# 1005088h/3d_object_detection

Hardware: AMD Instinct MI355X
Metric: point-cloud frames/sec end-to-end (voxelise→NMS), eight_20cm, 1x MI355X (higher is better)
Workload: dtype f32; 1 GPU; configs/eight_20cm.json, synthetic KITTI-shape 64-beam 20k-point clouds (mean 20000 points, one distinct cloud per frame of a step), independent frames (batch=1 semantics), random-init weights (InstanceNorm backbone), AABB NMS; `value`: clouds resident in HBM; frames_per_pass_per_gpu=32, engine_max_batch=32, parallelism=frame-sharded x1

## Files before the change

3d_object_detection_amd/_lib.py:

```python
import ctypes
import os

_HERE = os.path.dirname(os.path.abspath(__file__))
LIB_PATH = os.path.join(_HERE, "csrc", "libpp_hip.so")
PP_MAX_CLASSES = 12
PP_LOSS_TERMS = 21
PP_ASSIGN_MAX_GT = 4096
PP_AUG_MAX_BOXES = 256
PP_AUG_MAX_TRIES = 128
PP_AUG_PARAMS = 16
PP_OPT_CHUNK = 2048
PP_OPT_GROUP = 32

c_f = ctypes.c_float
c_i32 = ctypes.c_int32
c_i64 = ctypes.c_int64
c_p = ctypes.c_void_p


class PPConfig(ctypes.Structure):
    _fields_ = [
        ("voxel_size", c_f * 3),
        ("offset", c_f * 3),
        ("grid_size", c_i32 * 3),
# ... 12 lines not shown
        ("nms_iou_threshold", c_f),
        ("score_threshold", c_f),
        ("max_batch", c_i32),
    ]


PROTOTYPES = {
    "pp_create": (c_p, [ctypes.c_int, ctypes.POINTER(PPConfig)]),
    "pp_destroy": (None, [c_p]),
    "pp_last_error": (ctypes.c_char_p, [c_p]),
    "pp_load_weights": (ctypes.c_int, [c_p, ctypes.c_char_p, c_p, ctypes.POINTER(c_i64), ctypes.c_int]),
    "pp_commit_weights": (ctypes.c_int, [c_p]),
    "pp_set_precision": (ctypes.c_int, [c_p, ctypes.c_int]),
    "pp_effective_precision": (ctypes.c_int, [c_p]),
    "pp_set_anchors": (ctypes.c_int, [c_p, c_p, c_p, c_i64]),
    "pp_voxelize": (ctypes.c_int, [c_p, c_p, ctypes.c_int, ctypes.c_int, c_p, c_p, c_p, c_p, c_p]),
    "pp_anchor_mask": (ctypes.c_int, [c_p, c_p, c_p, c_p, c_p]),
    "pp_pfn": (ctypes.c_int, [c_p, c_p, c_p, c_p, c_p, c_p, c_p]),
    "pp_scatter": (ctypes.c_int, [c_p, c_p, c_p, c_p, c_p, c_p]),
    "pp_backbone": (ctypes.c_int, [c_p, c_p, c_p, c_p]),
    "pp_head": (ctypes.c_int, [c_p, c_p, c_p, c_p, c_p, c_p]),
    "pp_postprocess": (ctypes.c_int, [c_p, c_p, c_p, c_p, c_p, c_p, c_p, ctypes.c_int, c_p]),
    "pp_select_candidates": (ctypes.c_int, [c_p, c_p, c_p, c_p, c_p, c_p, c_p, c_p, c_p]),
    "pp_infer_frame": (ctypes.c_int, [c_p, c_p, ctypes.c_int, c_p, c_p, ctypes.c_int, c_p]),
    "pp_infer_batch": (ctypes.c_int, [c_p, ctypes.POINTER(c_p), ctypes.POINTER(c_i32), ctypes.c_int, c_p, c_p, ctypes.c_int, c_p]),
    "pp_fetch_frame_tensor": (ctypes.c_int, [c_p, ctypes.c_int, ctypes.c_int, c_p, c_p]),
    "pp_debug_layer": (ctypes.c_int, [c_p, ctypes.c_int, ctypes.c_int, c_p, c_p, ctypes.c_int, c_p, c_p, c_p, c_p, c_p, c_p, c_p, c_p, c_p]),
    "pp_debug_layer_skip": (ctypes.c_int, [c_p, ctypes.c_int, ctypes.c_int, c_p, c_p, ctypes.c_int, c_p, c_p, c_p, c_p, c_p, c_p, c_p, c_p, c_p, ctypes.c_int, c_p]),
    "pp_debug_head_cls": (ctypes.c_int, [c_p, ctypes.c_int, c_p, ctypes.c_int, c_p, c_p, c_p, c_p]),
    "pp_head_cls_tiling": (ctypes.c_char_p, [c_p]),
    "pp_set_head_defer": (ctypes.c_int, [c_p, ctypes.c_int]),
    "pp_head_defer_active": (ctypes.c_int, [c_p]),
    "pp_set_sparse_conv1": (ctypes.c_int, [c_p, ctypes.c_int]),
    "pp_set_tile_skip": (ctypes.c_int, [c_p, ctypes.c_int]),
    "pp_tile_skip_active": (ctypes.c_int, [c_p]),
    "pp_set_assign_thresholds": (ctypes.c_int, [c_p, c_p, c_p]),
    "pp_assign_targets": (ctypes.c_int, [c_p, c_p, c_p, c_p, ctypes.POINTER(c_i32), ctypes.c_int, c_p, c_p, c_p, c_p, c_p]),
    "pp_target_loss": (ctypes.c_int, [c_p, c_p, c_p, c_p, c_p, c_p, c_p, ctypes.c_int, c_p, c_p]),
    "pp_batch_loss": (ctypes.c_int, [c_p, c_p, c_p, ctypes.POINTER(c_i32), ctypes.c_int, c_p, c_p]),
    "pp_target_loss_grad": (ctypes.c_int, [c_p, c_p, c_p, c_p, c_p, c_p, c_p, ctypes.c_int, ctypes.c_int, c_f, c_p, c_p, c_p, c_p]),
    "pp_head_backward": (ctypes.c_int, [c_p, c_p, c_p, c_p, c_p, ctypes.c_int, c_p, c_p, c_p, c_p, c_p, c_p, c_p, c_p]),
    "pp_update_head_weights": (ctypes.c_int, [c_p, c_p, c_p, c_p, c_p, c_p, c_p, c_p]),
    "pp_backbone_taps": (ctypes.c_int, [c_p, c_p, c_p, c_p, c_p, c_p, c_p]),
    "pp_neck_backward": (ctypes.c_int, [c_p, ctypes.c_int, c_p, c_p, c_p, c_p, ctypes.c_int, c_p, c_p, c_p]),
    "pp_update_neck_weights": (ctypes.c_int, [c_p, c_p, c_p, c_p, c_p]),
    "pp_unit_backward": (ctypes.c_int, [c_p, ctypes.c_int, ctypes.c_int, ctypes.c_int, c_p, c_p, c_p, c_p, ctypes.c_int, c_p, c_p, c_p]),
    "pp_unit_backward_mp": (ctypes.c_int, [c_p, ctypes.c_int, ctypes.c_int, ctypes.c_int, ctypes.c_int, c_p, c_p, c_p, c_p, ctypes.c_int, c_p, c_p,
                                           c_p]),
    "pp_unit_backward_path": (ctypes.c_int, [c_p, ctypes.c_int, ctypes.c_int, ctypes.c_int, ctypes.c_int]),
    "pp_backbone_block_taps": (ctypes.c_int, [c_p, c_p, c_p, c_p, c_p, c_p, c_p, c_p]),
    "pp_update_block_weights": (ctypes.c_int, [c_p, ctypes.c_int, c_p, ctypes.c_int, c_p]),
    "pp_down_backward": (ctypes.c_int, [c_p, ctypes.c_int, ctypes.c_int, ctypes.c_int, ctypes.c_int, c_p, c_p, c_p, c_p, ctypes.c_int, c_p, c_p, c_p]),
    "pp_backbone_stage_taps": (ctypes.c_int, [c_p, c_p, c_p, c_p, c_p, c_p, c_p, c_p, c_p]),
    "pp_update_down_weight": (ctypes.c_int, [c_p, ctypes.c_int, c_p, c_p]),
    "pp_backbone_train_taps": (ctypes.c_int, [c_p, c_p, c_p, c_p, c_p, c_p, c_p, c_p, c_p]),
    "pp_update_rpn_weights": (ctypes.c_int, [c_p, c_p, c_p]),
    "pp_unit_backward_affine": (ctypes.c_int, [c_p, ctypes.c_int, ctypes.c_int, ctypes.c_int, c_p, c_p, c_p, c_p, c_p, c_p, ctypes.c_int, c_p, c_p, c_p,
                                               c_p, c_p]),
    "pp_down_backward_affine": (ctypes.c_int, [c_p, ctypes.c_int, ctypes.c_int, ctypes.c_int, ctypes.c_int, c_p, c_p, c_p, c_p, c_p, c_p, ctypes.c_int,
                                               c_p, c_p, c_p, c_p, c_p]),
    "pp_neck_backward_affine": (ctypes.c_int, [c_p, ctypes.c_int, c_p, c_p, c_p, c_p, c_p, c_p, ctypes.c_int, c_p, c_p, c_p, c_p, c_p]),
    "pp_bn_fold": (ctypes.c_int, [c_p, ctypes.c_int, c_p, c_p, c_p, c_p, c_p, c_p, c_p]),
    "pp_bn_affine_grad": (ctypes.c_int, [c_p, ctypes.c_int, c_p, c_p, c_p, c_p, c_p, c_p, c_p]),
    "pp_update_bn_fold": (ctypes.c_int, [c_p, c_p, c_p]),
    "pp_pfn_train_forward": (ctypes.c_int, [c_p] * 12),
    "pp_scatter_backward": (ctypes.c_int, [c_p] * 6),
# ... 65 lines not shown
```

3d_object_detection_amd/csrc/conv_inspect.hip:

```cpp
#include <algorithm>
#include <cstdio>
#include <cstring>
#include "conv_net.h"

using namespace ppc;

static int packed_indices(pp_ctx* ctx, const Layer& L, bool index_positions, std::vector<int32_t>& map)
{
    Layer scratch = L;
    scratch.w = nullptr;
    int rc = pack_layer(ctx, scratch, index_positions);
    if (rc) { if (scratch.w) (void)hipFree(scratch.w); return rc; }
    std::vector<float> image(scratch.w_bytes / sizeof(float));
    const hipError_t e = hipMemcpy(image.data(), scratch.w, scratch.w_bytes, hipMemcpyDeviceToHost);
    (void)hipFree(scratch.w);
    PP_HIP(e);
    map.resize(image.size());
    for (size_t i = 0; i < image.size(); ++i) map[i] = (int32_t)image[i] - 1;
    return 0;
}

static int layer_index_map(pp_ctx* ctx, const Layer& L, const std::vector<std::string>& names, std::vector<int32_t>& wmap)
{
    std::vector<std::vector<float>> saved(names.size());
// ... 86 lines not shown
        return 0;
    }
    return pp_fail(ctx, PP_E_ARG, "pp_net_deconv_image: no such upsampler");
}

extern "C" int pp_fetch_frame_tensor(pp_ctx* ctx, int frame, int kind, void* dst, void* stream_)
{
    if (!ctx || !dst) return pp_fail(ctx, PP_E_ARG, "pp_fetch_frame_tensor: null pointer");
    if (frame < 0 || frame >= ctx->max_batch) return pp_fail(ctx, PP_E_ARG, "pp_fetch_frame_tensor: frame out of range");
    hipStream_t stream = (hipStream_t)stream_;
    pp_net* net = (pp_net*)ctx->net;
    const size_t A = (size_t)ctx->A, mv = (size_t)ctx->cfg.max_voxels, HW = (size_t)ctx->H * ctx->W;
    const void* src = nullptr;
    size_t bytes = 0;
    if (kind == 1 || kind == 2)
        if (int rc0 = pp_head_materialise(ctx, stream)) return rc0;
    switch (kind) {
    case 0: src = ctx->f_cls + frame * A; bytes = A * 4; break;
    case 1: src = ctx->f_box + frame * A * 7; bytes = A * 28; break;
    case 2: src = ctx->f_dir + frame * A * 2; bytes = A * 8; break;
    case 3: src = ctx->f_mask + frame * A; bytes = A; break;
    case 4: {
        NormRef pre = norm_ref(ctx, 7, 320, 0, HW);
        if (pre.mode == PRE_STATS) pre.acc += (size_t)frame * STAT_FS;
        const float* src_ = net->up16 ? reinterpret_cast<const float*>(reinterpret_cast<const _Float16*>(net->up) + (size_t)frame * 320 * HW)
                                      : net->up + (size_t)frame * 320 * HW;
        return launch_norm_relu(ctx, src_, (float*)dst, 320, (int)HW, pre, nullptr, stream, 1, net->up16 ? 1 : 0);
    }
    case 5: src = ctx->f_feat + frame * mv * 64; bytes = mv * 64 * 4; break;
    case 6: src = ctx->f_coors + frame * mv * 3; bytes = mv * 12; break;
    case 7: src = ctx->f_num + frame * 4; bytes = 4; break;
    case 8: return pp_sc1_fetch_list(ctx, frame, dst, stream);
    case 9: return pp_ts_fetch_flags(ctx, frame, dst, stream);
    default: return pp_fail(ctx, PP_E_ARG, "pp_fetch_frame_tensor: unknown kind");
    }
    PP_HIP(hipMemcpyAsync(dst, src, bytes, hipMemcpyDeviceToDevice, stream));
    return 0;
}

namespace {
__global__ void __launch_bounds__(256) dbg_reduce_stats(const double* __restrict__ acc, size_t acc_fs, int C, double* __restrict__ out)
{
    const int i = blockIdx.x * 256 + threadIdx.x;
    if (i >= 2 * C) return;
    const double* a = acc + (size_t)blockIdx.y * acc_fs;
    double s = 0.0;
#pragma unroll
    for (int r = 0; r < NREP; ++r) s += a[(size_t)r * C * 2 + i];
    out[(size_t)blockIdx.y * 2 * C + i] = s;
}
}

extern "C" int pp_debug_layer(pp_ctx* ctx, int layer, int nb, const void* in, const void* res, int pre_mode, const float* scale, const float* shift,
                              const int32_t* pmap, const float* feat, void* out, float* out_box, float* out_dir, double* stats, void* stream_)
{
    return pp_debug_layer_skip(ctx, layer, nb, in, res, pre_mode, scale, shift, pmap, feat, out, out_box, out_dir, stats, nullptr, 0, stream_);
}

extern "C" int pp_debug_layer_skip(pp_ctx* ctx, int layer, int nb, const void* in, const void* res, int pre_mode, const float* scale, const float* shift,
                                   const int32_t* pmap, const float* feat, void* out, float* out_box, float* out_dir, double* stats,
                                   const uint8_t* active, int skip_k, void* stream_)
{
    if (!ctx) return PP_E_ARG;
    if (!ctx->net || !ctx->weights_ready) return pp_fail(ctx, PP_E_STATE, "pp_debug_layer: weights not committed");
    pp_net* net = (pp_net*)ctx->net;
    if (layer < 0 || layer >= (int)net->layers.size()) return pp_fail(ctx, PP_E_ARG, "pp_debug_layer: layer index out of range");
// ... 201 lines not shown
```

3d_object_detection_amd/csrc/conv_run.hip:

```cpp
#include <cstring>
#include "conv_net.h"

namespace ppc {
namespace {

__global__ void __launch_bounds__(256) norm_relu_stats(const float* __restrict__ x, float* __restrict__ y, int C, int HW,
                                                       int pre, const double* __restrict__ pre_acc,
                                                       const float* __restrict__ pre_scale, const float* __restrict__ pre_shift,
                                                       double inv_n, float eps, double* __restrict__ stat_acc,
                                                       size_t x_fs, size_t acc_fs, int x16, int y16)
{
    const int c = blockIdx.y;
    const _Float16* xh = reinterpret_cast<const _Float16*>(x) + blockIdx.z * x_fs;
    _Float16* yh = reinterpret_cast<_Float16*>(y) + blockIdx.z * x_fs;
    x += blockIdx.z * x_fs;
    y += blockIdx.z * x_fs;
    if (pre_acc) pre_acc += blockIdx.z * acc_fs;
    if (stat_acc) stat_acc += blockIdx.z * acc_fs;
    float sc, sh;
    if (pre == PRE_STATS) {
        double s = 0.0, q = 0.0;
        for (int r = 0; r < NREP; ++r) {
            s += pre_acc[((size_t)r * C + c) * 2];
            q += pre_acc[((size_t)r * C + c) * 2 + 1];
// ... 304 lines not shown

using namespace ppc;

static int run_upsampler(pp_ctx* ctx, const Layer& L, int b, const float* x, int nb, hipStream_t stream)
{
    pp_net* net = (pp_net*)ctx->net;
    const int H = ctx->H, W = ctx->W, coff = b == 0 ? 0 : b == 1 ? 64 : 192;
    double* st = stat_slot(ctx, 7);
    ConvCall k;
    k.in = x; k.Hin = k.Hout = H >> b; k.Win = k.Wout = W >> b;
    k.out = net->up16 ? reinterpret_cast<float*>(reinterpret_cast<_Float16*>(net->up) + (size_t)coff * H * W) : net->up + (size_t)coff * H * W;
    k.stat = st ? st + (size_t)coff * 2 : nullptr; k.stat_C = 320; k.nb = nb; k.out_fs = (size_t)320 * H * W;
    return launch_conv(ctx, L, k, stream);
}

int pp_run_backbone(pp_ctx* ctx, const float* canvas, int nb, hipStream_t stream, const int32_t* pmap, const float* feat)
{
    pp_net* net = (pp_net*)ctx->net;
    const int H = ctx->H, W = ctx->W;
    if ((H % 4) || (W % 4)) return pp_fail(ctx, PP_E_ARG, "backbone: BEV grid must be a multiple of 8 in x and y");
    if (nb < 1 || nb > ctx->max_batch) return pp_fail(ctx, PP_E_ARG, "backbone: batch exceeds cfg.max_batch");
    ctx->sc1_last_nb = 0;
    pp_ts_begin_pass(ctx);
    if (ctx->cfg.norm_kind == 0) PP_HIP(hipMemsetAsync(net->stats, 0, STAT_FS * sizeof(double) * nb, stream));
    const float* x = canvas;
    int Hin = ctx->gx, Win = ctx->gy;
    size_t li = 0;
    for (int b = 0; b < 3; ++b) {
        const int c = kC[b];
        const int h = H >> b, w = W >> b;
        const size_t cnt = (size_t)h * w;
        float** Bf = net->buf[b];
        int rc;
        if (b == 0 && pmap && net->eff_prec == 0 && pp_sc1_usable(ctx)) {
            ++li;
            if ((rc = pp_sc1_run(ctx, pmap, feat, Bf[0], stat_slot(ctx, site_block(0, 0)), STAT_FS, nb, stream))) return rc;
            if (ctx->sc1_last_nb == nb && !net->up16 && pp_ts_usable(ctx, 3) && level0_main_wino6(net, h, w)) {
                if ((rc = pp_ts_build(ctx, nb, nullptr, stream))) return rc;
                pp_ts_mark_pass(ctx, nb);
            }
        } else {
            ConvCall k;
            k.in = x; k.Hin = Hin; k.Win = Win; k.out = Bf[0]; k.Hout = h; k.Wout = w;
            k.stat = stat_slot(ctx, site_block(b, 0)); k.stat_C = c; k.nb = nb;
            if (b == 0) { k.pmap = pmap; k.feat = feat; }
            if ((rc = launch_conv(ctx, net->layers[li++], k, stream))) return rc;
        }
        if (nb == 1 && net->z_tap[b])
            PP_HIP(hipMemcpyAsync(net->z_tap[b], Bf[0], (size_t)c * cnt * sizeof(float), hipMemcpyDeviceToDevice, stream));
        if ((rc = pp_stage_mark(ctx, stream, PP_ST_NORM))) return rc;
        if ((rc = launch_norm_relu(ctx, Bf[0], Bf[1], c, (int)cnt, norm_ref(ctx, site_block(b, 0), c, 0, cnt),
                                   stat_slot(ctx, site_block(b, 1)), stream, nb, net->up16 ? 1 : 0, net->up16 ? 1 : 0))) return rc;
        if ((rc = pp_stage_mark(ctx, stream, PP_ST_CONV))) return rc;
        float* cur = Bf[1];
        float* spare[3] = {Bf[0], Bf[2], Bf[3]};
        float* utap = nb == 1 ? net->unit_tap[b] : nullptr;
        const size_t ubytes = (size_t)c * cnt * sizeof(float);
        int ucount = 0;
        if (utap) PP_HIP(hipMemcpyAsync(utap + (size_t)ucount++ * c * cnt, cur, ubytes, hipMemcpyDeviceToDevice, stream));
        int ts_k = 0;
        auto conv = [&](const float* in, float* out, const float* res, int site, double* stat) {
            ConvCall k;
            k.in = in; k.Hin = h; k.Win = w; k.out = out; k.Hout = h; k.Wout = w;
            k.res = res; k.pre = norm_ref(ctx, site_block(b, site), c, 0, cnt); k.stat = stat; k.stat_C = c;
            k.nb = nb; k.ts_k = b == 0 ? ++ts_k : 0;
            return launch_conv(ctx, net->layers[li++], k, stream);
        };
        for (int u = 0; u < block_units(b); ++u) {
            float* t1 = spare[0];
            float* t2 = spare[1];
            double* out_stat = u == block_units(b) - 1 ? nullptr : stat_slot(ctx, site_block(b, 1 + 2 * (u + 1)));
            if (unit_two_convs(b, u)) {
                if ((rc = conv(cur, t1, nullptr, 1 + 2 * u, stat_slot(ctx, site_block(b, 2 + 2 * u))))) return rc;
                if (utap) PP_HIP(hipMemcpyAsync(utap + (size_t)ucount++ * c * cnt, t1, ubytes, hipMemcpyDeviceToDevice, stream));
                if ((rc = conv(t1, t2, cur, 2 + 2 * u, out_stat))) return rc;
                if (utap) PP_HIP(hipMemcpyAsync(utap + (size_t)ucount++ * c * cnt, t2, ubytes, hipMemcpyDeviceToDevice, stream));
                spare[1] = cur;
                cur = t2;
            } else {
                if ((rc = conv(cur, t1, cur, 1 + 2 * u, out_stat))) return rc;
                spare[0] = cur;
                cur = t1;
            }
        }
        net->tap[b] = cur;
        if ((rc = run_upsampler(ctx, net->layers[li++], b, cur, nb, stream))) return rc;
// ... 156 lines not shown
```

3d_object_detection_amd/csrc/pp_common.h:

```cpp
#pragma once
#include <hip/hip_runtime.h>
#include <stdint.h>
#include <map>
#include <string>
#include <vector>
#include "../../include/pp_hip.h"

#define PP_EMPTY 0x7F7F7F7F

#define PP_HIP(call)                                                         \
    do {                                                                     \
        hipError_t e_ = (call);                                              \
        if (e_ != hipSuccess) return pp_fail_hip(ctx, e_, #call, __FILE__, __LINE__); \
    } while (0)

#if defined(__HIP_DEVICE_COMPILE__)
#define PP_GP __attribute__((address_space(1)))
#else
#define PP_GP
#endif
#define PP_SET(dst, src) dst = (decltype(dst))(src)
struct pp_pre_frame {
    int32_t PP_GP *pt_cell, *cell_first, *wave_cnt, *pt_rank, *slots, *scalars, *occ;
    float PP_GP* voxels;
// ... 119 lines not shown
int pp_fail_hip(pp_ctx* ctx, hipError_t e, const char* what, const char* file, int line);
int pp_fail(pp_ctx* ctx, int code, const char* msg);

int pp_net_create(pp_ctx* ctx);
void pp_net_destroy(pp_ctx* ctx);
int pp_net_commit(pp_ctx* ctx);
int pp_post_create(pp_ctx* ctx);
int pp_run_backbone(pp_ctx* ctx, const float* canvas, int nb, hipStream_t stream, const int32_t* pmap, const float* feat);
int pp_pillar_map(pp_ctx* ctx, const int32_t* coors, const int32_t* num_pillars, int32_t* pmap, hipStream_t stream);
int pp_build_tables(pp_ctx* ctx);
void pp_post_fill_table(pp_ctx* ctx, int slot, pp_post_frame* f);
int pp_voxelize_group(pp_ctx* ctx, int b0, int g, const pp_in_group& in, hipStream_t stream);
int pp_anchor_mask_group(pp_ctx* ctx, int b0, int g, hipStream_t stream);
int pp_pfn_pmap_group(pp_ctx* ctx, int b0, int g, hipStream_t stream);
int pp_postprocess_group(pp_ctx* ctx, int b0, int g, float* det, int32_t* det_count, int nms_mode, hipStream_t stream,
                         int defer_nb = 0);
int pp_run_head_fused(pp_ctx* ctx, float* cls, float* box, float* dir, int nb, hipStream_t stream);
bool pp_head_defer_on(pp_ctx* ctx);
int pp_run_head_cls(pp_ctx* ctx, float* cls, int nb, hipStream_t stream);
int pp_head_materialise(pp_ctx* ctx, hipStream_t stream);
struct pp_head_gather {
    const float* w; int bm, bmp, K;
    const float* bias_perm;
    const float* in; size_t in_fs; int HW;
    int pre; const double* pre_acc; size_t pre_fs; double pre_inv_n; const float *pre_scale, *pre_shift; size_t aff_fs; float eps;
};
int pp_net_head_gather(pp_ctx* ctx, int nb, pp_head_gather* g);
int pp_sc1_create(pp_ctx* ctx);
void pp_sc1_destroy(pp_ctx* ctx);
int pp_sc1_commit(pp_ctx* ctx);
int pp_sc1_update(pp_ctx* ctx, const float* w, hipStream_t stream);
const float* pp_first_conv_image(pp_ctx* ctx, size_t* bytes);
bool pp_sc1_usable(pp_ctx* ctx);
int pp_sc1_run(pp_ctx* ctx, const int32_t* pmap, const float* feat, float* out, double* stat, size_t stat_fs, int nb, hipStream_t stream);
int pp_sc1_fetch_list(pp_ctx* ctx, int frame, void* dst, hipStream_t stream);
const uint64_t* pp_sc1_words(pp_ctx* ctx, int* nblk);
int pp_ts_create(pp_ctx* ctx);
void pp_ts_destroy(pp_ctx* ctx);
bool pp_ts_usable(pp_ctx* ctx, int level0_layers);
void pp_ts_begin_pass(pp_ctx* ctx);
int pp_ts_build(pp_ctx* ctx, int nb, const uint64_t* words, hipStream_t stream);
int pp_ts_build_from_bitmap(pp_ctx* ctx, int nb, const uint8_t* bitmap, hipStream_t stream);
void pp_ts_mark_pass(pp_ctx* ctx, int nb);
void pp_ts_begin_hook(pp_ctx* ctx, bool builds);
void pp_ts_end_hook(pp_ctx* ctx);
bool pp_ts_list(pp_ctx* ctx, int k, int nb, const int2** items, const int32_t** count);
int pp_ts_fill(pp_ctx* ctx, int k, int nb, float* out, size_t out_fs, int C, hipStream_t stream);
int pp_ts_dense_items(pp_ctx* ctx, int nb);
int pp_ts_read_count(pp_ctx* ctx, int k, int32_t* n);
int pp_ts_fetch_flags(pp_ctx* ctx, int frame, void* dst, hipStream_t stream);
void pp_post_destroy(pp_ctx* ctx);
void pp_assign_destroy(pp_ctx* ctx);
void pp_train_destroy(pp_ctx* ctx);
struct pp_head_image {
    float *w = nullptr, *bias = nullptr, *bias_perm = nullptr;
    std::vector<int32_t> wmap, bmap, bpmap;
};
int pp_net_head_image(pp_ctx* ctx, pp_head_image* img);
struct pp_layer_image {
    float* w = nullptr;
    size_t elems = 0;
    std::vector<int32_t> wmap;
};
int pp_net_deconv_image(pp_ctx* ctx, int branch, pp_layer_image* img);
void pp_neck_destroy(pp_ctx* ctx);
struct pp_block_image {
    float* w = nullptr;
    int C = 0, T = 0;
// ... 12 lines not shown
```

3d_object_detection_amd/csrc/sparse_conv1.hip:

```cpp
#include <algorithm>
#include <cstring>
#include "pp_common.h"
#include "conv_common.h"

namespace {

using namespace ppc;

constexpr unsigned SC1_PARK = 0x80000000u;
constexpr int SC1_NT = 4;
constexpr int SC1_WAVE_PX = 16 * SC1_NT;
constexpr int SC1_W_FLOATS = 9 * 64 * 64;

struct Sc1 {
    float* w = nullptr;
    int kc = 4;
    uint64_t* words = nullptr;
    int32_t* bcnt = nullptr;
    int32_t* list = nullptr;
    uint32_t* tab = nullptr;
    int32_t* count = nullptr;
    int cap = 0, cap_pad = 0, nblk = 0;
    bool weights = false;
};

struct Sc1P {
    const int32_t* pmap; size_t pmap_fs;
    const float* feat; size_t feat_fs; unsigned feat_bytes;
    const float* w;
    float* out; size_t out_fs;
    double* stat; size_t stat_fs;
    uint64_t* words; int32_t* bcnt; int32_t* list; uint32_t* tab; int32_t* count;
    int Hin, Win, Hout, Wout, cap, cap_pad, nblk, max_voxels;
};

__global__ void __launch_bounds__(256) sc1_ballot_b(const Sc1P p)
{
    __shared__ int wc[4];
    const int f = blockIdx.z;
    const int32_t* __restrict__ gmap = p.pmap + (size_t)f * p.pmap_fs;
    const int pix = blockIdx.x * 256 + threadIdx.x;
    bool act = false;
    if (pix < p.Hout * p.Wout) {
        const int oy = pix / p.Wout, ox = pix - oy * p.Wout;
#pragma unroll
        for (int ky = 0; ky < 3; ++ky) {
            const int iy = 2 * oy - 1 + ky;
#pragma unroll
            for (int kx = 0; kx < 3; ++kx) {
                const int ix = 2 * ox - 1 + kx;
                if (iy >= 0 && iy < p.Hin && ix >= 0 && ix < p.Win) act |= gmap[(size_t)iy * p.Win + ix] >= 0;
            }
        }
    }
    const uint64_t b = __ballot(act);
    const int wave = threadIdx.x >> 6;
// ... 114 lines not shown

    const unsigned plane_b = (unsigned)(p.Hout * p.Wout) * 4u;
    const __amdgpu_buffer_rsrc_t ro = __builtin_amdgcn_make_buffer_rsrc(p.out + (size_t)f * p.out_fs, 0, plane_b * 64u, 0x00020000);
#pragma unroll
    for (int t = 0; t < NT; ++t) {
        const unsigned pix = __builtin_amdgcn_raw_buffer_load_b32(rl, eo[t], 0, 0);
        const unsigned oo = valid[t] ? pix * 4u + (unsigned)kq * 4u * plane_b : SC1_PARK;
#pragma unroll
        for (int i = 0; i < 4; ++i)
#pragma unroll
            for (int r = 0; r < 4; ++r) {
                const float x = acc[i][t][r];
                __builtin_amdgcn_raw_buffer_store_b32(__builtin_bit_cast(unsigned, x), ro, oo, (unsigned)(i * 16 + r) * plane_b, 0);
            }
    }
    if (p.stat) {
        double* __restrict__ gs = p.stat + (size_t)f * p.stat_fs + (size_t)(wv % NREP) * 64 * 2;
#pragma unroll
        for (int i = 0; i < 4; ++i)
#pragma unroll
            for (int r = 0; r < 4; ++r) {
                double s = 0.0, q = 0.0;
#pragma unroll
                for (int t = 0; t < NT; ++t) { const float x = acc[i][t][r]; const float xx = x * x; s += (double)x; q += (double)xx; }
#pragma unroll
                for (int d = 1; d < 16; d <<= 1) { s += __shfl_xor(s, d); q += __shfl_xor(q, d); }
                if (n == 0) {
                    double* dst = gs + (size_t)(i * 16 + kq * 4 + r) * 2;
                    atomicAdd(dst, s);
                    atomicAdd(dst + 1, q);
                }
            }
    }
}

template <int KC>
__global__ void __launch_bounds__(256) first_conv_image(const float* __restrict__ w, float* __restrict__ img)
{
    const int e = blockIdx.x * 256 + threadIdx.x;
    if (e >= SC1_W_FLOATS) return;
    const int i = e & 3, lane = (e >> 2) & 63, q = e >> 8;
    const int co = 16 * i + (lane & 15), ci = 4 * sc1_c4<KC>(q) + (lane >> 4);
    img[e] = w[((size_t)co * 64 + ci) * 9 + sc1_tap<KC>(q)];
}

template <typename T>
hipError_t sc1_alloc(T** q, size_t count) { return hipMalloc((void**)q, count * sizeof(T) + 256); }

}

int pp_sc1_create(pp_ctx* ctx)
{
    Sc1* S = new Sc1();
    ctx->sc1 = S;
    const size_t HW = (size_t)ctx->H * ctx->W, mb = (size_t)ctx->max_batch;
    const size_t cap = std::min((size_t)4 * ctx->cfg.max_voxels, HW);
    S->cap = (int)cap;
    S->cap_pad = (int)((cap + SC1_WAVE_PX - 1) / SC1_WAVE_PX) * SC1_WAVE_PX;
    S->nblk = pp_div_up((int64_t)HW, 256);
    PP_HIP(sc1_alloc(&S->w, (size_t)SC1_W_FLOATS));
    PP_HIP(sc1_alloc(&S->words, mb * S->nblk * 4));
    PP_HIP(sc1_alloc(&S->bcnt, mb * S->nblk));
    PP_HIP(sc1_alloc(&S->list, mb * S->cap_pad));
    PP_HIP(sc1_alloc(&S->tab, mb * 9 * S->cap_pad));
    PP_HIP(sc1_alloc(&S->count, mb));
    PP_HIP(hipMemset(S->list, 0, mb * S->cap_pad * sizeof(int32_t)));
    PP_HIP(hipMemset(S->tab, 0, mb * 9 * S->cap_pad * sizeof(uint32_t)));
    PP_HIP(hipMemset(S->count, 0, mb * sizeof(int32_t)));
    return 0;
}

void pp_sc1_destroy(pp_ctx* ctx)
{
    Sc1* S = (Sc1*)ctx->sc1;
    if (!S) return;
    void* ptrs[] = {S->w, S->words, S->bcnt, S->list, S->tab, S->count};
    for (void* q : ptrs)
        if (q) (void)hipFree(q);
    delete S;
    ctx->sc1 = nullptr;
}

int pp_sc1_commit(pp_ctx* ctx)
{
    Sc1* S = (Sc1*)ctx->sc1;
    S->weights = false;
    auto it = ctx->host_w.find("rpn.block1.0.weight");
    if (it == ctx->host_w.end() || it->second.data.size() != (size_t)SC1_W_FLOATS)
        return pp_fail(ctx, PP_E_NAME, "missing/mis-shaped weight rpn.block1.0.weight");
    const std::vector<float>& w = it->second.data;
    std::vector<float> img((size_t)SC1_W_FLOATS);
    S->kc = ctx->sc1_kc == 8 ? 8 : 4;
    for (int q = 0; q < 144; ++q) {
        const int c4 = S->kc == 8 ? sc1_c4<8>(q) : sc1_c4<4>(q), tap = S->kc == 8 ? sc1_tap<8>(q) : sc1_tap<4>(q);
        for (int lane = 0; lane < 64; ++lane)
            for (int i = 0; i < 4; ++i) {
                const int co = 16 * i + (lane & 15), ci = 4 * c4 + (lane >> 4);
                img[((size_t)q * 64 + lane) * 4 + i] = w[((size_t)co * 64 + ci) * 9 + tap];
            }
    }
    PP_HIP(hipMemcpy(S->w, img.data(), img.size() * sizeof(float), hipMemcpyHostToDevice));
    S->weights = true;
    return 0;
}

int pp_sc1_update(pp_ctx* ctx, const float* w, hipStream_t stream)
{
    Sc1* S = (Sc1*)ctx->sc1;
    if (!S || !S->weights) return 0;
    hipLaunchKernelGGL(S->kc == 8 ? first_conv_image<8> : first_conv_image<4>, dim3(pp_div_up(SC1_W_FLOATS, 256)), dim3(256), 0, stream, w, S->w);
    PP_HIP(hipGetLastError());
    return 0;
}

const float* pp_first_conv_image(pp_ctx* ctx, size_t* bytes)
{
    const Sc1* S = (const Sc1*)ctx->sc1;
    if (!S || !S->weights) return nullptr;
    *bytes = (size_t)SC1_W_FLOATS * sizeof(float);
    return S->w;
}

bool pp_sc1_usable(pp_ctx* ctx)
{
    const Sc1* S = (const Sc1*)ctx->sc1;
    return ctx->sparse_conv1 && S && S->weights && (size_t)64 * ctx->H * ctx->W * 4 < 0x7F000000ull &&
           (size_t)ctx->cfg.max_voxels * 256 < 0x7F000000ull;
}

int pp_sc1_run(pp_ctx* ctx, const int32_t* pmap, const float* feat, float* out, double* stat, size_t stat_fs, int nb, hipStream_t stream)
{
    Sc1* S = (Sc1*)ctx->sc1;
    const size_t HW = (size_t)ctx->H * ctx->W;
    ctx->sc1_last_nb = 0;
    PP_HIP(hipMemsetAsync(out, 0, (size_t)nb * 64 * HW * sizeof(float), stream));
    for (int b0 = 0; b0 < nb; b0 += PP_GROUP) {
        const int g = nb - b0 < PP_GROUP ? nb - b0 : PP_GROUP;
        Sc1P p;
        memset(&p, 0, sizeof(p));
        p.pmap_fs = (size_t)ctx->gx * ctx->gy; p.pmap = pmap + b0 * p.pmap_fs;
        p.feat_fs = (size_t)ctx->cfg.max_voxels * 64; p.feat = feat + b0 * p.feat_fs;
        p.feat_bytes = (unsigned)(p.feat_fs * 4);
        p.w = S->w;
        p.out_fs = 64 * HW; p.out = out + b0 * p.out_fs;
        p.stat_fs = stat_fs; p.stat = stat ? stat + b0 * stat_fs : nullptr;
        p.words = S->words + (size_t)b0 * S->nblk * 4; p.bcnt = S->bcnt + (size_t)b0 * S->nblk;
        p.list = S->list + (size_t)b0 * S->cap_pad; p.tab = S->tab + (size_t)b0 * 9 * S->cap_pad; p.count = S->count + b0;
        p.Hin = ctx->gx; p.Win = ctx->gy; p.Hout = ctx->H; p.Wout = ctx->W;
        p.cap = S->cap; p.cap_pad = S->cap_pad; p.nblk = S->nblk; p.max_voxels = ctx->cfg.max_voxels;
        hipLaunchKernelGGL(sc1_ballot_b, dim3(S->nblk, 1, g), dim3(256), 0, stream, p);
        hipLaunchKernelGGL(sc1_write_b, dim3(S->nblk, 1, g), dim3(256), 0, stream, p);
        hipLaunchKernelGGL(S->kc == 8 ? sc1_gather<8> : sc1_gather<4>, dim3(pp_div_up(S->cap_pad, 4 * SC1_WAVE_PX), 1, g), dim3(256), 0, stream, p);
    }
    PP_HIP(hipGetLastError());
    ctx->sc1_last_nb = nb;
    return 0;
}

int pp_sc1_fetch_list(pp_ctx* ctx, int frame, void* dst, hipStream_t stream)
{
    const Sc1* S = (const Sc1*)ctx->sc1;
    if (!S || frame >= ctx->sc1_last_nb) return pp_fail(ctx, PP_E_STATE, "pp_fetch_frame_tensor: the last pass did not build an active list for this frame");
    PP_HIP(hipMemcpyAsync(dst, S->count + frame, sizeof(int32_t), hipMemcpyDeviceToDevice, stream));
    PP_HIP(hipMemcpyAsync((int32_t*)dst + 1, S->list + (size_t)frame * S->cap_pad, (size_t)S->cap * sizeof(int32_t), hipMemcpyDeviceToDevice, stream));
    return 0;
}

const uint64_t* pp_sc1_words(pp_ctx* ctx, int* nblk)
{
    const Sc1* S = (const Sc1*)ctx->sc1;
    if (!S || ctx->sc1_last_nb < 1) return nullptr;
    *nblk = S->nblk;
    return S->words;
}

extern "C" int pp_set_sparse_conv1(pp_ctx* ctx, int on)
{
    if (!ctx) return PP_E_ARG;
    ctx->sparse_conv1 = on && !ctx->sparse_conv1_env_off;
    return 0;
}
```

3d_object_detection_amd/engine.py:

```python
import ctypes
import os
import re
import weakref

import numpy as np
import torch

from . import _lib

F32 = np.float32

DETECT_CLASSES = ["vehicle", "pedestrian", "cyclist"]
CLASS_TABLE = {
    "vehicle": dict(sizes=[[4.6, 2.10, 1.8], [7.5, 2.6, 2.9], [12.6, 2.9, 3.8]], rotations=[0, 1.5707963267948966],
                    matched_threshold=0.6, unmatched_threshold=0.45),
    "pedestrian": dict(sizes=[[0.96874749, 0.9645992, 1.81212425]], rotations=[0],
                       matched_threshold=0.45, unmatched_threshold=0.25),
    "cyclist": dict(sizes=[[2.02032733, 0.98075615, 1.72027404]], rotations=[0, 1.5707963267948966],
                    matched_threshold=0.5, unmatched_threshold=0.25),
}
NUM_ANCHOR_PER_LOC = 9


def class_table_of(config):
# ... 165 lines not shown

    def __del__(self):
        try:
            if getattr(self, "ctx", None):
                self.lib.pp_destroy(self.ctx)
                self.ctx = None
        except Exception:
            pass

    def set_precision(self, mode):
        if mode not in self.PRECISIONS:
            raise ValueError(f"precision must be one of {sorted(self.PRECISIONS)}")
        _lib.check(self.lib.pp_set_precision(self.ctx, self.PRECISIONS[mode]), self.ctx, "pp_set_precision")
        changed = mode != self.precision
        self.precision = mode
        if changed and self.weights_loaded:
            with torch.cuda.device(self.device):
                _lib.check(self.lib.pp_commit_weights(self.ctx), self.ctx, "pp_commit_weights")

    def effective_precision(self):
        v = self.lib.pp_effective_precision(self.ctx)
        return None if v < 0 else {n: k for k, n in self.PRECISIONS.items()}[v]

    def set_head_defer(self, on):
        _lib.check(self.lib.pp_set_head_defer(self.ctx, 1 if on else 0), self.ctx, "pp_set_head_defer")
        self.head_defer = bool(on) and not self._defer_env_off

    def head_defer_active(self):
        return bool(self.lib.pp_head_defer_active(self.ctx))

    def set_sparse_conv1(self, on):
        _lib.check(self.lib.pp_set_sparse_conv1(self.ctx, 1 if on else 0), self.ctx, "pp_set_sparse_conv1")

    def set_tile_skip(self, on):
        _lib.check(self.lib.pp_set_tile_skip(self.ctx, 1 if on else 0), self.ctx, "pp_set_tile_skip")

    def tile_skip_active(self):
        return bool(self.lib.pp_tile_skip_active(self.ctx))

    def load_state_dict(self, sd):
        for k, v in sd.items():
            if k.endswith("num_batches_tracked"):
                continue
            a = v.detach().cpu().numpy() if isinstance(v, torch.Tensor) else np.asarray(v)
            a = np.ascontiguousarray(a, dtype=F32)
            shape = (ctypes.c_int64 * max(a.ndim, 1))(*a.shape)
            _lib.check(self.lib.pp_load_weights(self.ctx, k.encode(), a.ctypes.data_as(ctypes.c_void_p), shape, a.ndim),
                       self.ctx, "pp_load_weights(" + k + ")")
        with torch.cuda.device(self.device):
            _lib.check(self.lib.pp_commit_weights(self.ctx), self.ctx, "pp_commit_weights")
        self.weights_loaded = True

    def _t(self, shape, dtype):
        return torch.empty(shape, dtype=dtype, device=self.device)

    def num_tensor(self, p):
        return torch.full((1,), int(p), dtype=torch.int32, device=self.device)

    def _on_device(self, who, named):
        for t, what in named:
            if t is not None and t.device != self.device:
                raise ValueError(f"{who}: {what} is on {t.device}, the engine on {self.device}")

    def _chk_weights(self, who, params, keys, shapes):
        out = []
        for k, shape in zip(keys, shapes):
# ... 600 lines not shown
        m = mask.view(torch.uint8) if mask.dtype == torch.bool else mask
        cls = _chk(cls.reshape(-1), torch.float32, (self.A,), "select_candidates: cls_preds")
        box = _chk(box.reshape(-1), torch.float32, (self.A * 7,), "select_candidates: box_preds")
        dr = _chk(dr.reshape(-1), torch.float32, (self.A * 2,), "select_candidates: dir_preds")
        m = _chk(m.reshape(-1), torch.uint8, (self.A,), "select_candidates: anchors_mask")
        with torch.cuda.device(self.device):
            _lib.check(self.lib.pp_select_candidates(self.ctx, _ptr(cls), _ptr(box), _ptr(dr), _ptr(m), _ptr(idx), _ptr(score), _ptr(count),
                                                     _stream()), self.ctx, "pp_select_candidates")
        return idx, score, count

    def infer_frame(self, points, det=None, cnt=None, nms_mode=0):
        if det is None:
            det = torch.zeros((self.cfg.num_classes * self.cfg.nms_post_max, 9), dtype=torch.float32, device=self.device)
            cnt = torch.zeros((1 + _lib.PP_MAX_CLASSES,), dtype=torch.int32, device=self.device)
        with torch.cuda.device(self.device):
            _lib.check(self.lib.pp_infer_frame(self.ctx, _ptr(points), int(points.shape[0]), _ptr(det), _ptr(cnt), int(nms_mode),
                                               _stream()), self.ctx, "pp_infer_frame")
        return det, cnt

    def infer_batch(self, points_list, det=None, cnt=None, nms_mode=0):
        nb = len(points_list)
        rows = self.cfg.num_classes * self.cfg.nms_post_max
        if det is None:
            det = torch.zeros((nb, rows, 9), dtype=torch.float32, device=self.device)
            cnt = torch.zeros((nb, 1 + _lib.PP_MAX_CLASSES), dtype=torch.int32, device=self.device)
        ptrs = (ctypes.c_void_p * nb)(*[p.data_ptr() if p.numel() else _ptr(p).value for p in points_list])
        ns = (ctypes.c_int32 * nb)(*[int(p.shape[0]) for p in points_list])
        with torch.cuda.device(self.device):
            _lib.check(self.lib.pp_infer_batch(self.ctx, ptrs, ns, nb, _ptr(det), _ptr(cnt), int(nms_mode), _stream()),
                       self.ctx, "pp_infer_batch")
        return det, cnt

    def fetch(self, frame, what):
        kinds = {"cls": (0, (self.A,), torch.float32), "box": (1, (self.A, 7), torch.float32), "dir": (2, (self.A, 2), torch.float32),
                 "mask": (3, (self.A,), torch.uint8), "rpn": (4, (320, self.H, self.W), torch.float32),
                 "feat": (5, (self.max_voxels, 64), torch.float32), "coors": (6, (self.max_voxels, 3), torch.int32),
                 "num": (7, (1,), torch.int32), "active": (8, (1 + min(4 * self.max_voxels, self.H * self.W),), torch.int32),
                 "tile_flags": (9, (3, self.H // 16, self.W // 16), torch.uint8)}
        kind, shape, dtype = kinds[what]
        out = torch.empty(shape, dtype=dtype, device=self.device)
        with torch.cuda.device(self.device):
            _lib.check(self.lib.pp_fetch_frame_tensor(self.ctx, int(frame), kind, _ptr(out), _stream()), self.ctx, "pp_fetch_frame_tensor")
        return out

    def debug_layer(self, layer, x=None, res=None, scale=None, shift=None, pmap=None, feat=None, stats=False, active=None, skip_k=0):
        til = self.layer_tilings()
        if not self.weights_loaded or not til:
            raise RuntimeError("debug_layer: load_state_dict first")
        if not isinstance(layer, int) or not 0 <= layer < len(til):
            raise ValueError(f"debug_layer: layer must be 0 .. {len(til) - 1}")
        t = til[layer]
        in_dt, out_dt = self.layer_io_dtypes(layer)
        kind, cin, cout, up = t["kind"], t["cin"], t["cout"], t["up"]
        h, w = self.H >> t["level"], self.W >> t["level"]
        s = 2 if kind == 0 and t["stride"] == 2 else 1
        hin, win = h * s, w * s
        sparse = pmap is not None or feat is not None
        if sparse:
            if layer != 0 or x is not None or pmap is None or feat is None:
                raise ValueError("debug_layer: the sparse form is pmap + feat, without x, on layer 0")
            nb = int(pmap.shape[0]) if isinstance(pmap, torch.Tensor) and pmap.dim() == 3 else 0
        else:
            nb = int(x.shape[0]) if isinstance(x, torch.Tensor) and x.dim() == 4 else 0
        if not 1 <= nb <= self.max_batch:
            raise ValueError(f"debug_layer: the input must hold 1 .. max_batch ({self.max_batch}) frames")
        if sparse:
            pmap = _chk(pmap, torch.int32, (nb, hin, win), "debug_layer: pmap")
            feat = _chk(feat, torch.float32, (nb, self.max_voxels, 64), "debug_layer: feat")
            xin = None
        else:
            x = _chk(x, in_dt, (nb, cin, hin, win), "debug_layer: x")
# ... 357 lines not shown
```

include/pp_hip.h:

```cpp
#ifndef PP_HIP_H
#define PP_HIP_H
#include <stdint.h>

#ifdef __cplusplus
extern "C" {
#endif

#define PP_MAX_CLASSES 12
#define PP_E_ARG 1
#define PP_E_STATE 2
#define PP_E_NAME 3

typedef struct pp_ctx pp_ctx;

typedef struct pp_config {
    float voxel_size[3];
    float offset[3];
    int32_t grid_size[3];
    int32_t max_voxels;
    int32_t max_num_points;
    int32_t num_point_features;
    int32_t max_points;
    int32_t num_anchor_per_loc;
    int32_t num_classes;
// ... 33 lines not shown

int pp_backbone(pp_ctx* ctx, const float* canvas, float* rpn_out, void* stream);

int pp_head(pp_ctx* ctx, const float* rpn_out, float* cls, float* box, float* dir, void* stream);

int pp_postprocess(pp_ctx* ctx, const float* cls, const float* box, const float* dir, const uint8_t* mask,
                   float* det, int32_t* det_count, int nms_mode, void* stream);

int pp_select_candidates(pp_ctx* ctx, const float* cls, const float* box, const float* dir, const uint8_t* mask,
                         int32_t* idx, float* score, int32_t* count, void* stream);

int pp_infer_frame(pp_ctx* ctx, const float* pts, int n, float* det, int32_t* det_count, int nms_mode, void* stream);

#define PP_DET_COUNT_STRIDE (1 + PP_MAX_CLASSES)
int pp_infer_batch(pp_ctx* ctx, const float* const* pts_h, const int32_t* n_h, int nb, float* det, int32_t* det_count,
                   int nms_mode, void* stream);

int pp_fetch_frame_tensor(pp_ctx* ctx, int frame, int kind, void* dst, void* stream);

int pp_debug_layer(pp_ctx* ctx, int layer, int nb, const void* in, const void* res, int pre_mode, const float* scale, const float* shift,
                   const int32_t* pmap, const float* feat, void* out, float* out_box, float* out_dir, double* stats, void* stream);

int pp_debug_layer_skip(pp_ctx* ctx, int layer, int nb, const void* in, const void* res, int pre_mode, const float* scale, const float* shift,
                        const int32_t* pmap, const float* feat, void* out, float* out_box, float* out_dir, double* stats,
                        const uint8_t* active, int skip_k, void* stream);

int pp_debug_head_cls(pp_ctx* ctx, int nb, const void* in, int pre_mode, const float* scale, const float* shift, float* cls_out, void* stream);
const char* pp_head_cls_tiling(pp_ctx* ctx);

int pp_set_head_defer(pp_ctx* ctx, int on);
int pp_head_defer_active(pp_ctx* ctx);

int pp_set_sparse_conv1(pp_ctx* ctx, int on);

int pp_set_tile_skip(pp_ctx* ctx, int on);
int pp_tile_skip_active(pp_ctx* ctx);

#define PP_ASSIGN_MAX_GT 4096
#define PP_LOSS_TERMS 21
int pp_set_assign_thresholds(pp_ctx* ctx, const float* matched_h, const float* unmatched_h);
int pp_assign_targets(pp_ctx* ctx, const uint8_t* mask, const float* gt, const int32_t* gt_cls, const int32_t* gt_off_h, int nb,
                      int32_t* labels, float* bbox_targets, float* outside_w, int32_t* dir_targets, void* stream);
int pp_target_loss(pp_ctx* ctx, const float* cls, const float* box, const float* dir, const int32_t* labels,
                   const float* bbox_targets, const int32_t* dir_targets, int nb, double* terms, void* stream);
int pp_batch_loss(pp_ctx* ctx, const float* gt, const int32_t* gt_cls, const int32_t* gt_off_h, int nb, double* terms, void* stream);

int pp_target_loss_grad(pp_ctx* ctx, const float* cls, const float* box, const float* dir, const int32_t* labels,
                        const float* bbox_targets, const int32_t* dir_targets, int nb, int batch_div, float grad_scale, float* dcls,
                        float* dbox, float* ddir, void* stream);
int pp_head_backward(pp_ctx* ctx, const float* rpn_out, const float* dcls, const float* dbox, const float* ddir, int nb, float* dw_cls,
                     float* dw_box, float* dw_dir, float* db_cls, float* db_box, float* db_dir, float* dx, void* stream);
int pp_update_head_weights(pp_ctx* ctx, const float* w_cls, const float* b_cls, const float* w_box, const float* b_box, const float* w_dir,
                           const float* b_dir, void* stream);

int pp_backbone_taps(pp_ctx* ctx, const float* canvas, float* rpn_out, float* x1, float* x2, float* x3, void* stream);
int pp_neck_backward(pp_ctx* ctx, int branch, const float* x, const float* w, const float* y, const float* dy, int nb, float* dw, float* dx,
                     void* stream);
int pp_update_neck_weights(pp_ctx* ctx, const float* w1, const float* w2, const float* w3, void* stream);

int pp_unit_backward(pp_ctx* ctx, int C, int h, int w, const float* u, const float* wgt, const float* dy, const float* dskip ,
                     int nb, float* dw, float* du , void* stream);
int pp_unit_backward_mp(pp_ctx* ctx, int mode, int C, int h, int w, const float* u, const float* wgt, const float* dy,
                        const float* dskip , int nb, float* dw, float* du , void* stream);
int pp_unit_backward_path(pp_ctx* ctx, int mode, int C, int h, int w);
int pp_backbone_block_taps(pp_ctx* ctx, const float* canvas, float* rpn_out, float* x1, float* x2, float* x3, float* units, void* stream);
int pp_update_block_weights(pp_ctx* ctx, int block, const float* const* w, int n, void* stream);
// ... 104 lines not shown
```

Before: 1091 frames/s.

## Keep a resident zeroed level-0 map and clear only written pixels after use

The sparse first convolution used to memset the whole 64-channel level-0 output for every batch before scattering into it. It now writes into a persistent buffer that is zeroed once. After the norm consumes it, a release kernel re-zeroes only the pixels listed as active, so per-pass memset bandwidth scales with occupied pixels instead of the full grid. This costs an extra max_batch×64×H×W allocation and relies on the active list covering every written pixel; debug fetch paths and a fill counter are added for verification.

```diff
diff --git a/3d_object_detection_amd/_lib.py b/3d_object_detection_amd/_lib.py
--- a/3d_object_detection_amd/_lib.py
+++ b/3d_object_detection_amd/_lib.py
@@ -68,6 +68,7 @@
     "pp_set_head_defer": (ctypes.c_int, [c_p, ctypes.c_int]),
     "pp_head_defer_active": (ctypes.c_int, [c_p]),
     "pp_set_sparse_conv1": (ctypes.c_int, [c_p, ctypes.c_int]),
+    "pp_sc1_full_fills": (ctypes.c_int, [c_p]),
     "pp_set_tile_skip": (ctypes.c_int, [c_p, ctypes.c_int]),
     "pp_tile_skip_active": (ctypes.c_int, [c_p]),
     "pp_set_assign_thresholds": (ctypes.c_int, [c_p, c_p, c_p]),
diff --git a/3d_object_detection_amd/csrc/conv_inspect.hip b/3d_object_detection_amd/csrc/conv_inspect.hip
--- a/3d_object_detection_amd/csrc/conv_inspect.hip
+++ b/3d_object_detection_amd/csrc/conv_inspect.hip
@@ -142,6 +142,8 @@
     case 7: src = ctx->f_num + frame * 4; bytes = 4; break;
     case 8: return pp_sc1_fetch_list(ctx, frame, dst, stream);
     case 9: return pp_ts_fetch_flags(ctx, frame, dst, stream);
+    case 10: return pp_sc1_fetch_nonzero(ctx, frame, dst, stream);
+    case 11: return pp_sc1_fetch_map(ctx, frame, dst, stream);
     default: return pp_fail(ctx, PP_E_ARG, "pp_fetch_frame_tensor: unknown kind");
     }
     PP_HIP(hipMemcpyAsync(dst, src, bytes, hipMemcpyDeviceToDevice, stream));
diff --git a/3d_object_detection_amd/csrc/conv_run.hip b/3d_object_detection_amd/csrc/conv_run.hip
--- a/3d_object_detection_amd/csrc/conv_run.hip
+++ b/3d_object_detection_amd/csrc/conv_run.hip
@@ -360,9 +360,11 @@
         const size_t cnt = (size_t)h * w;
         float** Bf = net->buf[b];
         int rc;
-        if (b == 0 && pmap && net->eff_prec == 0 && pp_sc1_usable(ctx)) {
+        const float* z = Bf[0];
+        const bool sparse = b == 0 && pmap && net->eff_prec == 0 && pp_sc1_usable(ctx);
+        if (sparse) {
             ++li;
-            if ((rc = pp_sc1_run(ctx, pmap, feat, Bf[0], stat_slot(ctx, site_block(0, 0)), STAT_FS, nb, stream))) return rc;
+            if ((rc = pp_sc1_run(ctx, pmap, feat, Bf[0], stat_slot(ctx, site_block(0, 0)), STAT_FS, nb, stream, &z))) return rc;
             if (ctx->sc1_last_nb == nb && !net->up16 && pp_ts_usable(ctx, 3) && level0_main_wino6(net, h, w)) {
                 if ((rc = pp_ts_build(ctx, nb, nullptr, stream))) return rc;
                 pp_ts_mark_pass(ctx, nb);
@@ -375,11 +377,12 @@
             if ((rc = launch_conv(ctx, net->layers[li++], k, stream))) return rc;
         }
         if (nb == 1 && net->z_tap[b])
-            PP_HIP(hipMemcpyAsync(net->z_tap[b], Bf[0], (size_t)c * cnt * sizeof(float), hipMemcpyDeviceToDevice, stream));
+            PP_HIP(hipMemcpyAsync(net->z_tap[b], z, (size_t)c * cnt * sizeof(float), hipMemcpyDeviceToDevice, stream));
         if ((rc = pp_stage_mark(ctx, stream, PP_ST_NORM))) return rc;
-        if ((rc = launch_norm_relu(ctx, Bf[0], Bf[1], c, (int)cnt, norm_ref(ctx, site_block(b, 0), c, 0, cnt),
+        if ((rc = launch_norm_relu(ctx, z, Bf[1], c, (int)cnt, norm_ref(ctx, site_block(b, 0), c, 0, cnt),
                                    stat_slot(ctx, site_block(b, 1)), stream, nb, net->up16 ? 1 : 0, net->up16 ? 1 : 0))) return rc;
         if ((rc = pp_stage_mark(ctx, stream, PP_ST_CONV))) return rc;
+        if (sparse && (rc = pp_sc1_release(ctx, nb, stream))) return rc;
         float* cur = Bf[1];
         float* spare[3] = {Bf[0], Bf[2], Bf[3]};
         float* utap = nb == 1 ? net->unit_tap[b] : nullptr;
diff --git a/3d_object_detection_amd/csrc/pp_common.h b/3d_object_detection_amd/csrc/pp_common.h
--- a/3d_object_detection_amd/csrc/pp_common.h
+++ b/3d_object_detection_amd/csrc/pp_common.h
@@ -175,8 +175,12 @@
 int pp_sc1_update(pp_ctx* ctx, const float* w, hipStream_t stream);
 const float* pp_first_conv_image(pp_ctx* ctx, size_t* bytes);
 bool pp_sc1_usable(pp_ctx* ctx);
-int pp_sc1_run(pp_ctx* ctx, const int32_t* pmap, const float* feat, float* out, double* stat, size_t stat_fs, int nb, hipStream_t stream);
+int pp_sc1_run(pp_ctx* ctx, const int32_t* pmap, const float* feat, float* fallback, double* stat, size_t stat_fs, int nb, hipStream_t stream,
+               const float** map);
+int pp_sc1_release(pp_ctx* ctx, int nb, hipStream_t stream);
 int pp_sc1_fetch_list(pp_ctx* ctx, int frame, void* dst, hipStream_t stream);
+int pp_sc1_fetch_nonzero(pp_ctx* ctx, int frame, void* dst, hipStream_t stream);
+int pp_sc1_fetch_map(pp_ctx* ctx, int frame, void* dst, hipStream_t stream);
 const uint64_t* pp_sc1_words(pp_ctx* ctx, int* nblk);
 int pp_ts_create(pp_ctx* ctx);
 void pp_ts_destroy(pp_ctx* ctx);
diff --git a/3d_object_detection_amd/csrc/sparse_conv1.hip b/3d_object_detection_amd/csrc/sparse_conv1.hip
--- a/3d_object_detection_amd/csrc/sparse_conv1.hip
+++ b/3d_object_detection_amd/csrc/sparse_conv1.hip
@@ -22,6 +22,10 @@
     int32_t* count = nullptr;
     int cap = 0, cap_pad = 0, nblk = 0;
     bool weights = false;
+    float* z = nullptr;
+    bool z_tried = false;
+    bool dirty = false;
+    int fills = 0;
 };
 
 struct Sc1P {
@@ -202,6 +206,33 @@
                 }
             }
     }
+}
+
+constexpr int SC1_REL_BLOCKS = 64;
+__global__ void __launch_bounds__(256) first_conv_release(const Sc1P p)
+{
+    const int f = blockIdx.z;
+    const int lane = threadIdx.x & 63, wave = threadIdx.x >> 6;
+    const int cnt = p.count[f];
+    const unsigned plane_b = (unsigned)(p.Hout * p.Wout) * 4u;
+    const __amdgpu_buffer_rsrc_t rl = __builtin_amdgcn_make_buffer_rsrc(p.list + (size_t)f * p.cap_pad, 0, (unsigned)p.cap_pad * 4u, 0x00020000);
+    const __amdgpu_buffer_rsrc_t ro = __builtin_amdgcn_make_buffer_rsrc(p.out + (size_t)f * p.out_fs, 0, plane_b * 64u, 0x00020000);
+    for (int e0 = (blockIdx.x * 4 + wave) * SC1_WAVE_PX; e0 < cnt; e0 += (int)gridDim.x * 4 * SC1_WAVE_PX) {
+        const bool valid = e0 + lane < cnt;
+        const unsigned pix = __builtin_amdgcn_raw_buffer_load_b32(rl, valid ? (unsigned)(e0 + lane) * 4u : SC1_PARK, 0, 0);
+        const unsigned oo = valid ? pix * 4u : SC1_PARK;
+#pragma unroll
+        for (int c = 0; c < 64; ++c) __builtin_amdgcn_raw_buffer_store_b32(0u, ro, oo, (unsigned)c * plane_b, 0);
+    }
+}
+
+__global__ void __launch_bounds__(256) first_conv_nonzero(const uint32_t* __restrict__ x, size_t n, int32_t* __restrict__ out)
+{
+    int c = 0;
+    for (size_t i = (size_t)blockIdx.x * 256 + threadIdx.x; i < n; i += (size_t)gridDim.x * 256) c += x[i] != 0u;
+#pragma unroll
+    for (int d = 1; d < 64; d <<= 1) c += __shfl_xor(c, d);
+    if ((threadIdx.x & 63) == 0 && c) atomicAdd(out, c);
 }
 
 template <int KC>
@@ -244,7 +275,7 @@
 {
     Sc1* S = (Sc1*)ctx->sc1;
     if (!S) return;
-    void* ptrs[] = {S->w, S->words, S->bcnt, S->list, S->tab, S->count};
+    void* ptrs[] = {S->w, S->words, S->bcnt, S->list, S->tab, S->count, S->z};
     for (void* q : ptrs)
         if (q) (void)hipFree(q);
     delete S;
@@ -298,32 +329,118 @@
            (size_t)ctx->cfg.max_voxels * 256 < 0x7F000000ull;
 }
 
-int pp_sc1_run(pp_ctx* ctx, const int32_t* pmap, const float* feat, float* out, double* stat, size_t stat_fs, int nb, hipStream_t stream)
+namespace {
+
+Sc1P sc1_params(const pp_ctx* ctx, const Sc1* S, const int32_t* pmap, const float* feat, float* out, double* stat, size_t stat_fs, int b0)
+{
+    const size_t HW = (size_t)ctx->H * ctx->W;
+    Sc1P p;
+    memset(&p, 0, sizeof(p));
+    p.pmap_fs = (size_t)ctx->gx * ctx->gy; p.pmap = pmap + b0 * p.pmap_fs;
+    p.feat_fs = (size_t)ctx->cfg.max_voxels * 64; p.feat = feat + b0 * p.feat_fs;
+    p.feat_bytes = (unsigned)(p.feat_fs * 4);
+    p.w = S->w;
+    p.out_fs = 64 * HW; p.out = out + b0 * p.out_fs;
+    p.stat_fs = stat_fs; p.stat = stat ? stat + b0 * stat_fs : nullptr;
+    p.words = S->words + (size_t)b0 * S->nblk * 4; p.bcnt = S->bcnt + (size_t)b0 * S->nblk;
+    p.list = S->list + (size_t)b0 * S->cap_pad; p.tab = S->tab + (size_t)b0 * 9 * S->cap_pad; p.count = S->count + b0;
+    p.Hin = ctx->gx; p.Win = ctx->gy; p.Hout = ctx->H; p.Wout = ctx->W;
+    p.cap = S->cap; p.cap_pad = S->cap_pad; p.nblk = S->nblk; p.max_voxels = ctx->cfg.max_voxels;
+    return p;
+}
+
+void sc1_launch(const Sc1* S, const Sc1P& p, int g, hipStream_t stream)
+{
+    hipLaunchKernelGGL(sc1_ballot_b, dim3(S->nblk, 1, g), dim3(256), 0, stream, p);
+    hipLaunchKernelGGL(sc1_write_b, dim3(S->nblk, 1, g), dim3(256), 0, stream, p);
+    hipLaunchKernelGGL(S->kc == 8 ? sc1_gather<8> : sc1_gather<4>, dim3(pp_div_up(S->cap_pad, 4 * SC1_WAVE_PX), 1, g), dim3(256), 0, stream, p);
+}
+
+int sc1_resident(pp_ctx* ctx, Sc1* S, hipStream_t stream)
+{
+    if (S->z_tried) return 0;
+    S->z_tried = true;
+    const size_t n = (size_t)ctx->max_batch * 64 * ctx->H * ctx->W;
+    if (sc1_alloc(&S->z, n) != hipSuccess) {
+        (void)hipGetLastError();
+        S->z = nullptr;
+        return 0;
+    }
+    PP_HIP(hipMemsetAsync(S->z, 0, n * sizeof(float), stream));
+    S->fills = 1;
+    return 0;
+}
+
+}
+
+int pp_sc1_run(pp_ctx* ctx, const int32_t* pmap, const float* feat, float* fallback, double* stat, size_t stat_fs, int nb, hipStream_t stream,
+               const float** map)
 {
     Sc1* S = (Sc1*)ctx->sc1;
     const size_t HW = (size_t)ctx->H * ctx->W;
     ctx->sc1_last_nb = 0;
-    PP_HIP(hipMemsetAsync(out, 0, (size_t)nb * 64 * HW * sizeof(float), stream));
+    if (int rc = sc1_resident(ctx, S, stream)) return rc;
+    float* out = S->z ? S->z : fallback;
+    if (!S->z) PP_HIP(hipMemsetAsync(out, 0, (size_t)nb * 64 * HW * sizeof(float), stream));
+    else if (S->dirty) {
+        PP_HIP(hipMemsetAsync(S->z, 0, (size_t)ctx->max_batch * 64 * HW * sizeof(float), stream));
+        ++S->fills;
+    }
+    S->dirty = S->z != nullptr;
     for (int b0 = 0; b0 < nb; b0 += PP_GROUP) {
         const int g = nb - b0 < PP_GROUP ? nb - b0 : PP_GROUP;
-        Sc1P p;
-        memset(&p, 0, sizeof(p));
-        p.pmap_fs = (size_t)ctx->gx * ctx->gy; p.pmap = pmap + b0 * p.pmap_fs;
-        p.feat_fs = (size_t)ctx->cfg.max_voxels * 64; p.feat = feat + b0 * p.feat_fs;
-        p.feat_bytes = (unsigned)(p.feat_fs * 4);
-        p.w = S->w;
-        p.out_fs = 64 * HW; p.out = out + b0 * p.out_fs;
-        p.stat_fs = stat_fs; p.stat = stat ? stat + b0 * stat_fs : nullptr;
-        p.words = S->words + (size_t)b0 * S->nblk * 4; p.bcnt = S->bcnt + (size_t)b0 * S->nblk;
-        p.list = S->list + (size_t)b0 * S->cap_pad; p.tab = S->tab + (size_t)b0 * 9 * S->cap_pad; p.count = S->count + b0;
-        p.Hin = ctx->gx; p.Win = ctx->gy; p.Hout = ctx->H; p.Wout = ctx->W;
-        p.cap = S->cap; p.cap_pad = S->cap_pad; p.nblk = S->nblk; p.max_voxels = ctx->cfg.max_voxels;
-        hipLaunchKernelGGL(sc1_ballot_b, dim3(S->nblk, 1, g), dim3(256), 0, stream, p);
-        hipLaunchKernelGGL(sc1_write_b, dim3(S->nblk, 1, g), dim3(256), 0, stream, p);
-        hipLaunchKernelGGL(S->kc == 8 ? sc1_gather<8> : sc1_gather<4>, dim3(pp_div_up(S->cap_pad, 4 * SC1_WAVE_PX), 1, g), dim3(256), 0, stream, p);
+        sc1_launch(S, sc1_params(ctx, S, pmap, feat, out, stat, stat_fs, b0), g, stream);
     }
     PP_HIP(hipGetLastError());
     ctx->sc1_last_nb = nb;
+    *map = out;
+    return 0;
+}
+
+int pp_sc1_release(pp_ctx* ctx, int nb, hipStream_t stream)
+{
+    Sc1* S = (Sc1*)ctx->sc1;
+    if (!S || !S->dirty) return 0;
+    for (int b0 = 0; b0 < nb; b0 += PP_GROUP) {
+        const int g = nb - b0 < PP_GROUP ? nb - b0 : PP_GROUP;
+        hipLaunchKernelGGL(first_conv_release, dim3(SC1_REL_BLOCKS, 1, g), dim3(256), 0, stream, sc1_params(ctx, S, nullptr, nullptr, S->z, nullptr, 0, b0));
+    }
+    PP_HIP(hipGetLastError());
+    S->dirty = false;
+    return 0;
+}
+
+extern "C" int pp_sc1_full_fills(pp_ctx* ctx)
+{
+    const Sc1* S = ctx ? (const Sc1*)ctx->sc1 : nullptr;
+    return S ? S->fills : 0;
+}
+
+int pp_sc1_fetch_nonzero(pp_ctx* ctx, int frame, void* dst, hipStream_t stream)
+{
+    const Sc1* S = (const Sc1*)ctx->sc1;
+    if (!S || !S->z) return pp_fail(ctx, PP_E_STATE, "pp_fetch_frame_tensor: the context holds no resident level-0 map (no sparse pass yet)");
+    const size_t n = (size_t)64 * ctx->H * ctx->W;
+    PP_HIP(hipMemsetAsync(dst, 0, sizeof(int32_t), stream));
+    const int blocks = (int)std::min<size_t>((n + 255) / 256, 1024);
+    hipLaunchKernelGGL(first_conv_nonzero, dim3(blocks), dim3(256), 0, stream, (const uint32_t*)(S->z + (size_t)frame * n), n, (int32_t*)dst);
+    PP_HIP(hipGetLastError());
+    return 0;
+}
+
+int pp_sc1_fetch_map(pp_ctx* ctx, int frame, void* dst, hipStream_t stream)
+{
+    Sc1* S = (Sc1*)ctx->sc1;
+    if (!S || frame >= ctx->sc1_last_nb) return pp_fail(ctx, PP_E_STATE, "pp_fetch_frame_tensor: the last pass did not run the sparse first conv for this frame");
+    if (!S->z || S->dirty) return pp_fail(ctx, PP_E_STATE, "pp_fetch_frame_tensor: no resident level-0 map to compute into");
+    const Sc1P p = sc1_params(ctx, S, ctx->f_pmap, ctx->f_feat, S->z, nullptr, 0, frame);
+    S->dirty = true;
+    sc1_launch(S, p, 1, stream);
+    PP_HIP(hipGetLastError());
+    PP_HIP(hipMemcpyAsync(dst, p.out, p.out_fs * sizeof(float), hipMemcpyDeviceToDevice, stream));
+    hipLaunchKernelGGL(first_conv_release, dim3(SC1_REL_BLOCKS, 1, 1), dim3(256), 0, stream, p);
+    PP_HIP(hipGetLastError());
+    S->dirty = false;
     return 0;
 }
 
diff --git a/3d_object_detection_amd/engine.py b/3d_object_detection_amd/engine.py
--- a/3d_object_detection_amd/engine.py
+++ b/3d_object_detection_amd/engine.py
@@ -221,6 +221,9 @@
     def set_sparse_conv1(self, on):
         _lib.check(self.lib.pp_set_sparse_conv1(self.ctx, 1 if on else 0), self.ctx, "pp_set_sparse_conv1")
 
+    def sc1_full_fills(self):
+        return int(self.lib.pp_sc1_full_fills(self.ctx))
+
     def set_tile_skip(self, on):
         _lib.check(self.lib.pp_set_tile_skip(self.ctx, 1 if on else 0), self.ctx, "pp_set_tile_skip")
 
@@ -887,11 +890,12 @@
         return det, cnt
 
     def fetch(self, frame, what):
-        kinds = {"cls": (0, (self.A,), torch.float32), "box": (1, (self.A, 7), torch.float32), "dir": (2, (self.A, 2), torch.float32),
+        kinds ={"cls": (0, (self.A,), torch.float32), "box": (1, (self.A, 7), torch.float32), "dir": (2, (self.A, 2), torch.float32),
                  "mask": (3, (self.A,), torch.uint8), "rpn": (4, (320, self.H, self.W), torch.float32),
                  "feat": (5, (self.max_voxels, 64), torch.float32), "coors": (6, (self.max_voxels, 3), torch.int32),
                  "num": (7, (1,), torch.int32), "active": (8, (1 + min(4 * self.max_voxels, self.H * self.W),), torch.int32),
-                 "tile_flags": (9, (3, self.H // 16, self.W // 16), torch.uint8)}
+                 "tile_flags": (9, (3, self.H // 16, self.W // 16), torch.uint8), "z_nonzero": (10, (1,), torch.int32),
+                 "z": (11, (64, self.H, self.W), torch.float32)}
         kind, shape, dtype = kinds[what]
         out = torch.empty(shape, dtype=dtype, device=self.device)
         with torch.cuda.device(self.device):
diff --git a/include/pp_hip.h b/include/pp_hip.h
--- a/include/pp_hip.h
+++ b/include/pp_hip.h
@@ -89,6 +89,7 @@
 int pp_head_defer_active(pp_ctx* ctx);
 
 int pp_set_sparse_conv1(pp_ctx* ctx, int on);
+int pp_sc1_full_fills(pp_ctx* ctx);
 
 int pp_set_tile_skip(pp_ctx* ctx, int on);
 int pp_tile_skip_active(pp_ctx* ctx);
```

Measured after the change: 1094 frames/s (median of 6 runs). Within noise of the previous version (+0.2%).
